# jason-li-831202/Vehicle-CV-ADAS

Hardware: AMD Instinct MI355X
Metric: frames/sec end-to-end (detect+lane+NMS+track) per GPU; conv MFMA util % (higher is better)
Workload: dtype fp16x3

## Files before the change

include/adas_hip.h:

```cpp
#ifndef ADAS_HIP_H
#define ADAS_HIP_H
#include <stddef.h>
#include <stdint.h>

#ifdef __cplusplus
extern "C" {
#endif

typedef enum {
    ADAS_OK = 0,
    ADAS_ERR_INVALID = -1,
    ADAS_ERR_IO = -2,
    ADAS_ERR_FORMAT = -3,
    ADAS_ERR_HIP = -4,
    ADAS_ERR_CAPACITY = -5,
    ADAS_ERR_NO_DEVICE = -6
} adas_status;

const char* adas_last_error(void);
int adas_version(void);
int adas_device_count(void);
int adas_set_device(int index);
int adas_device_pci_bus_id(int index, char* out, int out_len);
int adas_malloc(void** d_ptr, size_t bytes);
// ... 42 lines not shown
int adas_engine_ml_info(const adas_engine* e, int batch, int32_t* n_launches, int32_t* n_layers, int32_t* n_items);
int adas_engine_ml_status(const adas_engine* e, int batch, uint32_t* error_word);
int adas_engine_launch_count(adas_engine* e, int batch);
int adas_engine_ml_counters(const adas_engine* e, int batch, int launch, uint32_t head16[16]);
typedef struct adas_ml_view {
    uint64_t buf;
    int32_t cs, coff, c, h, w;
} adas_ml_view;
typedef struct adas_ml_layer_desc {
    int32_t kernel, stride, act, res_mode, up_c, halo_bn;
    adas_ml_view x, y, res, up;
} adas_ml_layer_desc;
int adas_debug_ml_plan(const adas_ml_layer_desc* layers, int n_layers, int batch, int precision, int32_t* deps, int32_t* targets,
                       uint64_t* items, int items_cap, int32_t summary[4]);
int adas_debug_conv_route(const adas_ml_layer_desc* layer, int batch, int precision, char* name, int name_cap);
#define ADAS_PLAN_COLS 29
int adas_engine_plan(const adas_engine* e, int64_t* rows, int rows_cap, int32_t* n_ops, uint64_t* weight_bytes);
int adas_debug_engine_plan(const void* tables, size_t bytes, int precision, int max_batch, int64_t* rows, int rows_cap, int32_t* n_ops,
                           uint64_t* weight_bytes);
#define ADAS_LABEL_CAP 96
int adas_engine_schedule(const adas_engine* e, int batch, int32_t* step_of, int32_t* role, int cap, int32_t* n_ops, int32_t* n_steps);
int adas_debug_engine_schedule(const void* tables, size_t bytes, int precision, int max_batch, int batch, int32_t* step_of, int32_t* role,
                               char* labels, int cap, int32_t* n_ops, int32_t* n_steps);
int adas_engine_fetch_activation(adas_engine* e, int layer, int batch, float* h_out_nchw, int64_t dims[4]);

int adas_preprocess_yolo(const uint8_t* d_frames_bgr, int n, int src_h, int src_w, float* d_out_nchw, int dst_h,
                         int dst_w, int keep_ratio, void* stream);
int adas_preprocess_ufld(const uint8_t* d_frames_bgr, int n, int src_h, int src_w, float* d_out_nchw, int in_h,
                         int in_w, double crop_ratio, void* stream);
int adas_preprocess_yolo_packed(const uint8_t* d_frames_bgr, int n, int src_h, int src_w, uint16_t* d_out_nhwc4, int dst_h,
// ... 507 lines not shown
```

vehicle-cv-adas_amd/_lib.py:

```python
import ctypes as C
import os

import numpy as np

HERE = os.path.dirname(os.path.abspath(__file__))
LIB_PATH = os.environ.get("ADAS_LIB") or os.path.join(HERE, "libadas_hip.so")

UFLD_MAX_POINTS = 128
HEAD_V8, HEAD_V5, HEAD_V5_LITE = 0, 1, 2
NMS_REFERENCE, NMS_GREEDY = 0, 1
PREC_BF16, PREC_FP32, PREC_FP16, PREC_FP16X3 = 0, 1, 2, 3
PRECISIONS = {"bf16": PREC_BF16, "fp32": PREC_FP32, "fp16": PREC_FP16, "fp16x3": PREC_FP16X3}


class AdasError(RuntimeError):
    def __init__(self, code, msg):
        super().__init__(f"libadas_hip error {code}: {msg}")
        self.code = code


class YoloPostParams(C.Structure):
    _fields_ = [("layout", C.c_int32), ("num_anchors", C.c_int32), ("num_classes", C.c_int32), ("nms_mode", C.c_int32),
                ("box_score", C.c_double), ("iou_thr", C.c_double), ("pad_h", C.c_int32), ("pad_w", C.c_int32),
                ("ratio_h", C.c_double), ("ratio_w", C.c_double), ("max_candidates", C.c_int32), ("reserved", C.c_int32)]
# ... 197 lines not shown
    "adas_engine_num_outputs": (C.c_int, [_P]),
    "adas_engine_output_shape": (C.c_int, [_P, C.c_int, C.POINTER(C.c_int64), C.POINTER(C.c_int)]),
    "adas_engine_output_name": (C.c_char_p, [_P, C.c_int]),
    "adas_engine_infer_host": (C.c_int, [_P, _P, C.c_int, C.POINTER(_P)]),
    "adas_engine_infer_device": (C.c_int, [_P, _P, C.c_int, _P]),
    "adas_engine_accepts_packed_input": (C.c_int, [_P]),
    "adas_engine_precision": (C.c_int, [_P]),
    "adas_engine_prepare": (C.c_int, [_P, C.c_int]),
    "adas_engine_ml_info": (C.c_int, [_P, C.c_int, C.POINTER(C.c_int32), C.POINTER(C.c_int32), C.POINTER(C.c_int32)]),
    "adas_engine_ml_status": (C.c_int, [_P, C.c_int, C.POINTER(C.c_uint32)]),
    "adas_engine_launch_count": (C.c_int, [_P, C.c_int]),
    "adas_engine_ml_counters": (C.c_int, [_P, C.c_int, C.c_int, C.POINTER(C.c_uint32)]),
    "adas_debug_ml_plan": (C.c_int, [C.POINTER(MlLayerDesc), C.c_int, C.c_int, C.c_int, C.POINTER(C.c_int32), C.POINTER(C.c_int32), C.POINTER(C.c_uint64),
                                     C.c_int, C.POINTER(C.c_int32)]),
    "adas_debug_conv_route": (C.c_int, [C.POINTER(MlLayerDesc), C.c_int, C.c_int, C.c_char_p, C.c_int]),
    "adas_engine_plan": (C.c_int, [_P, C.POINTER(C.c_int64), C.c_int, C.POINTER(C.c_int32), C.POINTER(C.c_uint64)]),
    "adas_debug_engine_plan": (C.c_int, [C.c_char_p, C.c_size_t, C.c_int, C.c_int, C.POINTER(C.c_int64), C.c_int, C.POINTER(C.c_int32), C.POINTER(C.c_uint64)]),
    "adas_engine_schedule": (C.c_int, [_P, C.c_int, C.POINTER(C.c_int32), C.POINTER(C.c_int32), C.c_int, C.POINTER(C.c_int32), C.POINTER(C.c_int32)]),
    "adas_debug_engine_schedule": (C.c_int, [C.c_char_p, C.c_size_t, C.c_int, C.c_int, C.c_int, C.POINTER(C.c_int32), C.POINTER(C.c_int32), C.c_char_p,
                                             C.c_int, C.POINTER(C.c_int32), C.POINTER(C.c_int32)]),
    "adas_engine_model_io_half": (C.c_int, [_P]),
    "adas_engine_infer_device_packed": (C.c_int, [_P, _P, C.c_int, _P]),
    "adas_engine_output_device": (_P, [_P, C.c_int]),
    "adas_engine_stats": (C.c_int, [_P, C.POINTER(C.c_double), C.POINTER(C.c_double), C.POINTER(C.c_int)]),
    "adas_engine_profile": (C.c_int, [_P, _P, C.c_int, C.c_int, _P, C.c_int, C.POINTER(C.c_int)]),
    "adas_engine_layer_info": (C.c_int, [_P, C.c_int, C.c_char_p, C.c_int, C.POINTER(C.c_double), C.POINTER(C.c_int)]),
    "adas_engine_layer_kernel": (C.c_int, [_P, C.c_int, C.c_int, C.c_char_p, C.c_int]),
    "adas_engine_fetch_activation": (C.c_int, [_P, C.c_int, C.c_int, _P, C.POINTER(C.c_int64)]),
    "adas_preprocess_yolo": (C.c_int, [_P, C.c_int, C.c_int, C.c_int, _P, C.c_int, C.c_int, C.c_int, _P]),
    "adas_preprocess_ufld": (C.c_int, [_P, C.c_int, C.c_int, C.c_int, _P, C.c_int, C.c_int, C.c_double, _P]),
# ... 257 lines not shown
```

vehicle-cv-adas_amd/csrc/conv_halo8_x3.hip:

```cpp
#include "kernels.h"
#include "elem16.h"
#include <stdlib.h>
#include <string.h>
#include <type_traits>

namespace adas {

typedef __attribute__((ext_vector_type(4))) float yf32x4;
typedef __attribute__((ext_vector_type(4))) uint32_t yu32x4;
typedef __attribute__((ext_vector_type(2))) uint32_t yu32x2;
typedef __attribute__((address_space(3))) void* ylds_vp;

struct H8XDev {
    const void* in;
    const void* wgt;
    const float* bias;
    void* out;
    const void* res;
    uint32_t in_bytes, wgt_bytes, out_bytes, res_bytes;
    int in_cs, in_coff, cin, H, W;
    int out_cs, out_coff, cout;
    int res_cs, res_coff, res_mode;
    int nck;
    int SW, NS, TPS, WW;
// ... 67 lines not shown
constexpr int X8_NBIAS = 2, X8_NRES = 8;
#endif

#ifdef ADAS_H8X_PROF
__device__ unsigned long long g_h8x_prof[256][32];
#define H8XP(i)                                     \
    if (lane == 0 && grp == 0) {                    \
        const unsigned long long t__ = clock64();   \
        pacc__[i] += t__ - tprev__;                 \
        tprev__ = t__;                              \
    }
#else
#define H8XP(i)
#endif

__host__ __device__ constexpr int x8s_issued(bool lo, int k, int nwp) { return ((lo ? k >= 3 : (k >= 0 && k < 3)) ? 1 : 0) + ((k >= 1 && k <= nwp) ? 1 : 0); }
__host__ __device__ constexpr int x8s_allow(bool lo, int k, int nwp) { return x8s_issued(lo, k, nwp) + x8s_issued(lo, k - 1, nwp) + x8s_issued(lo, k - 2, nwp); }

template <int ACT, int MODE, bool LH, bool SH, int NWP>
__global__ __launch_bounds__(X8_THR, 1) void conv_h8x3_kernel(H8XDev a) {
    static_assert(!SH || (MODE == 2 && !LH), "shared weight tiles: one barrier per tap row, whole tiles");
    static_assert(NWP >= 1 && NWP <= X8_NWP && (SH || NWP == X8_NWP), "window pieces per wave");
    Fp16::enter();
    typedef Fp16::vec8 hvec8;
    constexpr int LOOK = x8_look(MODE);
    extern __shared__ __attribute__((aligned(16))) uint8_t lds8[];

    const int tid = threadIdx.x, lane = tid & 63;
    const int wave = __builtin_amdgcn_readfirstlane(tid >> 6);
    const int lrow = lane & 15, kg = lane >> 4;
// ... 244 lines not shown
            tap(std::integral_constant<int, 3>{}); tap(std::integral_constant<int, 4>{}); tap(std::integral_constant<int, 5>{});
            tap(std::integral_constant<int, 6>{}); tap(std::integral_constant<int, 7>{}); tap(std::integral_constant<int, 8>{});
#ifdef ADAS_H8X_PROF
            if (lastc) { H8XP(3) } else if (islo) { H8XP(2) } else { H8XP(1) }
#endif
        };
        for (int c = 0; c + 1 < a.nck; ++c) {
            if (c & 1) chunk(std::false_type{}, std::true_type{}, c);
            else chunk(std::false_type{}, std::false_type{}, c);
        }
        chunk(std::true_type{}, std::true_type{}, a.nck - 1);

        __builtin_amdgcn_s_waitcnt(0x0F70);
        H8XP(4)
#if !defined(ADAS_H8X_SCALAR_EPI) && !defined(ADAS_H8X_NARROW_ST)
        auto write_out = [&](auto rm_c) {
            constexpr int RM = decltype(rm_c)::value;
            yf32x2 val[4][2][2];
#pragma unroll
            for (int j = 0; j < 4; ++j)
#pragma unroll
                for (int i = 0; i < 2; ++i) {
                    yf32x2 v0 = yf32x2{acc[i + 2][j][0], acc[i + 2][j][1]} * kX3Down + yf32x2{acc[i][j][0], acc[i][j][1]};
                    yf32x2 v1 = yf32x2{acc[i + 2][j][2], acc[i + 2][j][3]} * kX3Down + yf32x2{acc[i][j][2], acc[i][j][3]};
                    if (RM != RES_NONE) {
                        const auto q0 = __builtin_amdgcn_permlane16_swap(rraw[j][i].x, rraw[j][i].z, false, false);
                        const auto q1 = __builtin_amdgcn_permlane16_swap(rraw[j][i].y, rraw[j][i].w, false, false);
                        const yf32x2 r0 = x8_join2(q0[0], q0[1]), r1 = x8_join2(q1[0], q1[1]);
                        if (RM == RES_BEFORE_ACT) { v0 = x8_act2<ACT>(v0 + r0); v1 = x8_act2<ACT>(v1 + r1); }
                        else { v0 = x8_act2<ACT>(v0) + r0; v1 = x8_act2<ACT>(v1) + r1; }
                    } else {
                        v0 = x8_act2<ACT>(v0); v1 = x8_act2<ACT>(v1);
                    }
                    val[j][i][0] = v0; val[j][i][1] = v1;
                    acc[i][j] = yf32x4{biasn[i].x, biasn[i].y, biasn[i].z, biasn[i].w};
                    acc[i + 2][j] = yf32x4{0.f, 0.f, 0.f, 0.f};
                }
            uint32_t hw[4][2][2];
            x8_hi_mode(true);
#pragma unroll
            for (int j = 0; j < 4; ++j)
#pragma unroll
                for (int i = 0; i < 2; ++i) {
                    hw[j][i][0] = x8_cvt_hi2(val[j][i][0]);
                    hw[j][i][1] = x8_cvt_hi2(val[j][i][1]);
                }
            x8_hi_mode(false);
#pragma unroll
            for (int j = 0; j < 4; ++j) {
                const uint32_t oo = po[j] == X8_OOB ? X8_OOB : (po[j] * (uint32_t)a.out_cs + (uint32_t)a.out_coff) * 4u + ch0;
#pragma unroll
                for (int i = 0; i < 2; ++i) {
                    const uint32_t oi = (cb * 64 + hb * 32 + i * 16 + (kg >> 1) * 8 < a.cout) ? oo + i * 64 : X8_OOB;
                    const uint32_t l0 = x8_lo2(val[j][i][0], hw[j][i][0]), l1 = x8_lo2(val[j][i][1], hw[j][i][1]);
                    const auto s0 = __builtin_amdgcn_permlane16_swap(hw[j][i][0], l0, false, false);
                    const auto s1 = __builtin_amdgcn_permlane16_swap(hw[j][i][1], l1, false, false);
                    __builtin_amdgcn_raw_buffer_store_b128(yu32x4{s0[0], s1[0], s0[1], s1[1]}, rout, oi, 0, 0);
                }
            }
        };
#else
        auto write_out = [&](auto rm_c) {
            constexpr int RM = decltype(rm_c)::value;
#pragma unroll
            for (int j = 0; j < 4; ++j) {
                const uint32_t oo = po[j] == X8_OOB ? X8_OOB : (po[j] * (uint32_t)a.out_cs + (uint32_t)a.out_coff) * 4u + ch0;
#pragma unroll
                for (int i = 0; i < 2; ++i) {
#ifdef ADAS_H8X_NARROW_ST
                    const uint32_t oi = (cb * 64 + hb * 32 + i * 16 + kg * 4 < a.cout) ? oo + i * 64 : X8_OOB;
#else
                    const uint32_t oi = (cb * 64 + hb * 32 + i * 16 + (kg >> 1) * 8 < a.cout) ? oo + i * 64 : X8_OOB;
#endif
                    float v[4];
#pragma unroll
// ... 59 lines not shown
#pragma unroll
        for (int i = 0; i < NWP; ++i) gcur[i] = gnxt[i];
        wcur = wnxt_item;
        par = (par + a.nck) & 1;
    }
    if (MODE == 1 && !hb) __builtin_amdgcn_s_barrier();
#ifdef ADAS_H8X_PROF
    if (lane == 0 && grp == 0) {
        unsigned long long* b__ = g_h8x_prof[blockIdx.x & 255];
        for (int i__ = 0; i__ < 16; ++i__)
            if (i__ != 7) atomicAdd(&b__[i__ + 16 * hb], pacc__[i__]);
        atomicAdd(&b__[7 + 16 * hb], (unsigned long long)nit__);
    }
#endif
}

#ifdef ADAS_H8X_PROF
extern "C" int adas_debug_h8x_prof(unsigned long long* out32, int reset) {
    static unsigned long long h[256][32];
    if (out32) {
        if (hipMemcpyFromSymbol(h, HIP_SYMBOL(g_h8x_prof), sizeof(h)) != hipSuccess) return -1;
        for (int i = 0; i < 32; ++i) {
            out32[i] = 0;
            for (int b = 0; b < 256; ++b) out32[i] += h[b][i];
        }
    }
    if (reset) {
        memset(h, 0, sizeof(h));
        if (hipMemcpyToSymbol(HIP_SYMBOL(g_h8x_prof), h, sizeof(h)) != hipSuccess) return -1;
    }
// ... 130 lines not shown
    static bool attr_done = false;
    if (!attr_done) {
        (void)hipFuncSetAttribute((const void*)conv_h8x3_kernel<ACT_NONE, MODE, LH, false, X8_NWP>, hipFuncAttributeMaxDynamicSharedMemorySize, 160 * 1024);
        (void)hipFuncSetAttribute((const void*)conv_h8x3_kernel<ACT_SILU, MODE, LH, false, X8_NWP>, hipFuncAttributeMaxDynamicSharedMemorySize, 160 * 1024);
        (void)hipFuncSetAttribute((const void*)conv_h8x3_kernel<ACT_RELU, MODE, LH, false, X8_NWP>, hipFuncAttributeMaxDynamicSharedMemorySize, 160 * 1024);
        (void)hipFuncSetAttribute((const void*)conv_h8x3_kernel<ACT_LEAKY, MODE, LH, false, X8_NWP>, hipFuncAttributeMaxDynamicSharedMemorySize, 160 * 1024);
        attr_done = true;
    }
    if (act == ACT_SILU) hipLaunchKernelGGL((conv_h8x3_kernel<ACT_SILU, MODE, LH, false, X8_NWP>), grid, dim3(X8_THR), X8_LDS, st, d);
    else if (act == ACT_RELU) hipLaunchKernelGGL((conv_h8x3_kernel<ACT_RELU, MODE, LH, false, X8_NWP>), grid, dim3(X8_THR), X8_LDS, st, d);
    else if (act == ACT_LEAKY) hipLaunchKernelGGL((conv_h8x3_kernel<ACT_LEAKY, MODE, LH, false, X8_NWP>), grid, dim3(X8_THR), X8_LDS, st, d);
    else hipLaunchKernelGGL((conv_h8x3_kernel<ACT_NONE, MODE, LH, false, X8_NWP>), grid, dim3(X8_THR), X8_LDS, st, d);
    return hipGetLastError();
}

hipError_t launch_conv_halo8_x3(const ConvArgs& a, hipStream_t st) {
    HaloPlan pl;
    if (!a.wgt_h8x3 || !halo8_x3_applicable(a) || !x8_plan(a.out.h, a.out.w, &pl)) return hipErrorInvalidValue;
    {
        static int sw = -1;
        if (sw < 0) { const char* e = getenv("ADAS_H8X_SW"); sw = e ? atoi(e) : 0; }
        HaloPlan alt;
        if (sw > 0 && plan_halo_sw(a.out.h, a.out.w, 1, sw, X8_MAXPIX, &alt) && alt.eff >= 0.6) {
            const long nt = (long)a.n * alt.NS * alt.TPS;
            if (x8_blocks_per_unit((nt + 7) / 8, x8_cout_pad(a.out.c) / 64) > 0) pl = alt;
        }
    }
    H8XDev d;
    d.in = a.in.p; d.wgt = a.wgt_h8x3; d.bias = a.bias; d.out = a.out.p; d.res = a.res.p;
    d.in_cs = a.in.cs; d.in_coff = a.in.coff; d.cin = a.in.c; d.H = a.in.h; d.W = a.in.w;
    d.out_cs = a.out.cs; d.out_coff = a.out.coff; d.cout = a.out.c;
    d.res_cs = a.res.cs; d.res_coff = a.res.coff; d.res_mode = a.res_mode;
    d.nck = 2 * (x8_cin_pad(a.in.c) / 32);
    d.in_bytes = (uint32_t)((size_t)a.n * a.in.h * a.in.w * a.in.cs * 4);
    d.wgt_bytes = (uint32_t)halo8_x3_weight_bytes(a.out.c, a.in.c);
    d.out_bytes = (uint32_t)((size_t)a.n * a.out.h * a.out.w * a.out.cs * 4);
    d.res_bytes = a.res_mode != RES_NONE ? (uint32_t)((size_t)a.n * a.out.h * a.out.w * a.res.cs * 4) : 0u;
    d.SW = pl.SW; d.NS = pl.NS; d.TPS = pl.TPS; d.WW = pl.WW;
    d.mg_ww = pl.mg_ww; d.mg_sw = pl.mg_sw;
    d.mg_img = (uint32_t)(((1ull << 32) + (uint64_t)(pl.NS * pl.TPS) - 1) / (uint64_t)(pl.NS * pl.TPS));
    d.mg_tps = (uint32_t)(((1ull << 32) + (uint64_t)pl.TPS - 1) / (uint64_t)pl.TPS);
    d.ntiles = a.n * pl.NS * pl.TPS;
    d.tiles8 = (d.ntiles + 7) / 8;
    d.ncb = x8_cout_pad(a.out.c) / 64;
    d.cpw = x8_blocks_per_unit(d.tiles8, d.ncb);
    if (d.cpw <= 0) return hipErrorInvalidValue;
    const int upt = d.ncb / d.cpw;
    d.mg_upt = (uint32_t)(((1ull << 32) + (uint64_t)upt - 1) / (uint64_t)upt);
    const int units8 = d.tiles8 * upt;
    static int max_slots = -1;
    if (max_slots < 0) { const char* e = getenv("ADAS_H8X_SLOTS"); max_slots = e ? atoi(e) : X8_SLOTS; if (max_slots < 8 || max_slots > 4096) max_slots = X8_SLOTS; }
    const int slots = units8 < max_slots ? units8 : max_slots;
    dim3 grid(8 * slots);
    const int forced = x8_mode();
    const bool pingpong = forced == 3;
    if (x8_share() && forced != 3) {
        const int nwp = (pl.maxpix + 127) / 128;
        if (nwp <= 3) return x8_launch_sh<3>(d, a.act, grid, st);
        if (nwp == 4) return x8_launch_sh<4>(d, a.act, grid, st);
        return x8_launch_sh<5>(d, a.act, grid, st);
    }
    if (x8_lhalf()) return pingpong ? x8_launch<1, true>(d, a.act, grid, st) : x8_launch<2, true>(d, a.act, grid, st);
    return pingpong ? x8_launch<1, false>(d, a.act, grid, st) : x8_launch<2, false>(d, a.act, grid, st);
}

}
```

vehicle-cv-adas_amd/csrc/engine.cpp:

```cpp
#include "engine.h"
#include <string.h>
#include <string>
#include <vector>

using namespace adas;

int adas::free_engine(adas_engine* e) {
    if (!e) return ADAS_OK;
    for (auto& kv : e->schedules) free_schedule(&kv.second);
    e->schedules.clear();
    for (auto& b : e->bufs)
        if (b.d && b.alias_of < 0) (void)hipFree(b.d);
    if (e->d_weights) (void)hipFree(e->d_weights);
    if (e->d_input) (void)hipFree(e->d_input);
    for (auto& ev : e->events)
        if (ev) (void)hipEventDestroy(ev);
    delete e;
    return ADAS_OK;
}

extern "C" {

int adas_engine_destroy(adas_engine* e) { return free_engine(e); }

// ... 370 lines not shown
    }
    return ADAS_OK;
}

int adas_debug_conv_route(const adas_ml_layer_desc* layer, int batch, int precision, char* name, int name_cap) {
    ADAS_REQUIRE(layer && batch > 0 && precision >= PREC_BF16 && precision <= PREC_X3 && name && name_cap > 0, ADAS_ERR_INVALID,
                 "adas_debug_conv_route: bad argument");
    ConvArgs a = conv_args_of_desc(*layer, batch, precision);
    const ConvPlan pl = plan_conv(precision, a.kh, a.kw, a.stride, a.pad, a.max_n, a.res_mode, a.in, a.out);
    a.kpad = pl.kpad;
    if (wants_x3h8_packing(precision, pl.kernel, a.kh, a.kw, a.stride, a.pad, a.res_mode, a.in, a.out)) a.wgt_h8x3 = (const void*)(uintptr_t)0x1000;
    snprintf(name, name_cap, "%s", conv_kernel_name(a));
    return ADAS_OK;
}

int adas_engine_precision(const adas_engine* e) { return e ? e->prec : -1; }
int adas_engine_model_io_half(const adas_engine* e) { return e ? (int)((e->hdr.in_cpad >> 16) & 1u) : 0; }

int adas_engine_accepts_packed_input(const adas_engine* e) {
    return (e && e->prec != PREC_X3 && e->ops.size() >= 2 && e->ops[0].skip && e->ops[1].kernel == CONV_STEM) ? 1 : 0;
}

int adas_engine_infer_device_packed(adas_engine* e, const uint16_t* d_input_nhwc4, int batch, void* stream) {
    ADAS_REQUIRE(e && d_input_nhwc4 && batch > 0 && batch <= e->max_batch, ADAS_ERR_INVALID, "adas_engine_infer_device_packed: bad argument");
    ADAS_REQUIRE(adas_engine_accepts_packed_input(e), ADAS_ERR_INVALID,
                 "this engine's first layer is not the fused stem (fp32 mode or ADAS_NO_STEM): feed the fp32 NCHW tensor instead");
    e->last = (hipStream_t)stream;
    return engine_forward(e, reinterpret_cast<const float*>(d_input_nhwc4), batch, (hipStream_t)stream, true);
}

// ... 109 lines not shown
```

vehicle-cv-adas_amd/csrc/kernels.h:

```cpp
#pragma once
#include <hip/hip_runtime.h>
#include <stdint.h>

namespace adas {

enum { PREC_BF16 = 0, PREC_FP32 = 1, PREC_FP16 = 2, PREC_X3 = 3 };
inline bool prec_is16(int prec) { return prec == PREC_BF16 || prec == PREC_FP16; }
inline int prec_esize(int prec) { return prec_is16(prec) ? 2 : 4; }
enum { ACT_NONE = 0, ACT_SILU = 1, ACT_RELU = 2, ACT_LEAKY = 3 ,
       ACT_HSWISH = 4 , ACT_HSIGMOID = 5 , ACT_RELU6 = 6  };
enum { RES_NONE = 0, RES_AFTER_ACT = 1, RES_BEFORE_ACT = 2 };

int persist_slots(int which);

struct TView {
    void* p;
    int cs, coff, c;
    int h, w;
    int f32;
};

struct ConvArgs {
    TView in, out, res;
    const void* wgt;
// ... 65 lines not shown
hipError_t launch_conv_c2f16_x3(const TView& x, const TView& out, const void* const w[4], const float* const b[4], int n, hipStream_t st);
hipError_t launch_conv_c2f16(const TView& x, const TView& out, const void* w_cv1, const float* b_cv1, const void* w_a, const float* b_a, const void* w_b,
                             const float* b_b, const void* w_cv2, const float* b_cv2, int n, int prec, hipStream_t st);
bool pw_applicable(int prec, int kh, int kw, int stride, int pad, int res_mode, const TView& in, const TView& out);
bool pwg_applicable(const ConvArgs& a);
hipError_t launch_conv_pwg(const ConvArgs& a, hipStream_t st);
const char* pwg_kernel_name(int m, int cout);
hipError_t launch_conv_x3(const ConvArgs& a, hipStream_t st);
const char* conv_x3_kernel_name(const ConvArgs& a);
hipError_t launch_pack_weights_x3(const float* src, void* dst, int cout, int cout_pad, int taps, int cin, int cin_pad, int kpad, hipStream_t st);
bool halo8_x3_shape_ok(int kh, int kw, int stride, int pad, const TView& in, const TView& out);
bool halo8_x3_applicable(const ConvArgs& a);
size_t halo8_x3_weight_bytes(int cout, int cin);
hipError_t launch_pack_weights_h8x3(const float* src, void* dst, int cout, int cin, hipStream_t st);
hipError_t launch_conv_halo8_x3(const ConvArgs& a, hipStream_t st);
hipError_t launch_conv(const ConvArgs& a, hipStream_t st);
const char* conv_kernel_name(const ConvArgs& a, bool stem = false);

hipError_t launch_input_nchw(const float* nchw, TView out, int n, int c_true, int prec, hipStream_t st);
hipError_t launch_maxpool(TView in, TView out, int n, int k, int s, int p, int prec, hipStream_t st);
hipError_t launch_avgpool(TView in, TView out, int n, int k, int s, int p, int prec, hipStream_t st);
hipError_t launch_upsample2(TView in, TView out, int n, int prec, hipStream_t st);
bool depth2space_supported(const TView& in, const TView& out);
hipError_t launch_depth2space(TView in, TView out, int n, int prec, hipStream_t st);
hipError_t launch_detect_v6(const TView* ins, float* out, int n, int nc, int A, const int strides[3], hipStream_t st);
hipError_t launch_detect_v6_dfl(const TView* ins, float* out, int n, int nc, int A, const int strides[3], hipStream_t st);
bool sppf_pool3_applicable(int prec, const TView& in, const TView out[3]);
hipError_t launch_sppf_pool3(const TView& in, const TView out[3], int n, int prec, hipStream_t st);
hipError_t launch_detect_v8(const TView* ins, float* out, int n, int nc, int A, const int strides[3], hipStream_t st);
hipError_t launch_detect_v8_fused(const TView* hidden, const void* const* wfrag, const float* const* bias, float* out, int n, int nc, int A,
// ... 67 lines not shown
```

Measured before the change: 5562.

## Add one-pass halo8 x3 conv kernel with double-buffered input window

Adds a new 3x3 fp16x3 halo conv kernel variant that keeps two full input windows in LDS (up to 160 KB) and a six-slot weight ring. It streams the next tile's window and weights while the current chunk's MFMAs run, replacing the shared-window path for tiles of up to 384 pixels. The epilogue is moved into a shared device function. The aim is to hide input-window reload latency and cut barriers between tiles and channel blocks, at the cost of one block per CU from the large LDS footprint and more complex scheduling. It is on by default and can be disabled with an environment variable.

```diff
diff --git a/include/adas_hip.h b/include/adas_hip.h
--- a/include/adas_hip.h
+++ b/include/adas_hip.h
@@ -80,6 +80,7 @@
 int adas_debug_ml_plan(const adas_ml_layer_desc* layers, int n_layers, int batch, int precision, int32_t* deps, int32_t* targets,
                        uint64_t* items, int items_cap, int32_t summary[4]);
 int adas_debug_conv_route(const adas_ml_layer_desc* layer, int batch, int precision, char* name, int name_cap);
+int adas_debug_h8x3_onepass(const adas_ml_layer_desc* layer, int batch);
 #define ADAS_PLAN_COLS 29
 int adas_engine_plan(const adas_engine* e, int64_t* rows, int rows_cap, int32_t* n_ops, uint64_t* weight_bytes);
 int adas_debug_engine_plan(const void* tables, size_t bytes, int precision, int max_batch, int64_t* rows, int rows_cap, int32_t* n_ops,
diff --git a/vehicle-cv-adas_amd/_lib.py b/vehicle-cv-adas_amd/_lib.py
--- a/vehicle-cv-adas_amd/_lib.py
+++ b/vehicle-cv-adas_amd/_lib.py
@@ -235,6 +235,7 @@
     "adas_debug_ml_plan": (C.c_int, [C.POINTER(MlLayerDesc), C.c_int, C.c_int, C.c_int, C.POINTER(C.c_int32), C.POINTER(C.c_int32), C.POINTER(C.c_uint64),
                                      C.c_int, C.POINTER(C.c_int32)]),
     "adas_debug_conv_route": (C.c_int, [C.POINTER(MlLayerDesc), C.c_int, C.c_int, C.c_char_p, C.c_int]),
+    "adas_debug_h8x3_onepass": (C.c_int, [C.POINTER(MlLayerDesc), C.c_int]),
     "adas_engine_plan": (C.c_int, [_P, C.POINTER(C.c_int64), C.c_int, C.POINTER(C.c_int32), C.POINTER(C.c_uint64)]),
     "adas_debug_engine_plan": (C.c_int, [C.c_char_p, C.c_size_t, C.c_int, C.c_int, C.POINTER(C.c_int64), C.c_int, C.POINTER(C.c_int32), C.POINTER(C.c_uint64)]),
     "adas_engine_schedule": (C.c_int, [_P, C.c_int, C.POINTER(C.c_int32), C.POINTER(C.c_int32), C.c_int, C.POINTER(C.c_int32), C.POINTER(C.c_int32)]),
diff --git a/vehicle-cv-adas_amd/csrc/conv_halo8_x3.hip b/vehicle-cv-adas_amd/csrc/conv_halo8_x3.hip
--- a/vehicle-cv-adas_amd/csrc/conv_halo8_x3.hip
+++ b/vehicle-cv-adas_amd/csrc/conv_halo8_x3.hip
@@ -105,6 +105,55 @@
 #define H8XP(i)
 #endif
 
+#if !defined(ADAS_H8X_SCALAR_EPI) && !defined(ADAS_H8X_NARROW_ST)
+template <int ACT, int RM>
+__device__ __forceinline__ void x8_write_out(const H8XDev& a, __amdgpu_buffer_rsrc_t rout, yf32x4 (&acc)[4][4], const yu32x4 (&rraw)[4][2],
+                                             const float4 (&biasn)[2], const uint32_t (&po)[4], uint32_t ch0, int cb, int hb, int kg) {
+    yf32x2 val[4][2][2];
+#pragma unroll
+    for (int j = 0; j < 4; ++j)
+#pragma unroll
+        for (int i = 0; i < 2; ++i) {
+            yf32x2 v0 = yf32x2{acc[i + 2][j][0], acc[i + 2][j][1]} * kX3Down + yf32x2{acc[i][j][0], acc[i][j][1]};
+            yf32x2 v1 = yf32x2{acc[i + 2][j][2], acc[i + 2][j][3]} * kX3Down + yf32x2{acc[i][j][2], acc[i][j][3]};
+            if (RM != RES_NONE) {
+                const auto q0 = __builtin_amdgcn_permlane16_swap(rraw[j][i].x, rraw[j][i].z, false, false);
+                const auto q1 = __builtin_amdgcn_permlane16_swap(rraw[j][i].y, rraw[j][i].w, false, false);
+                const yf32x2 r0 = x8_join2(q0[0], q0[1]), r1 = x8_join2(q1[0], q1[1]);
+                if (RM == RES_BEFORE_ACT) { v0 = x8_act2<ACT>(v0 + r0); v1 = x8_act2<ACT>(v1 + r1); }
+                else { v0 = x8_act2<ACT>(v0) + r0; v1 = x8_act2<ACT>(v1) + r1; }
+            } else {
+                v0 = x8_act2<ACT>(v0); v1 = x8_act2<ACT>(v1);
+            }
+            val[j][i][0] = v0; val[j][i][1] = v1;
+            acc[i][j] = yf32x4{biasn[i].x, biasn[i].y, biasn[i].z, biasn[i].w};
+            acc[i + 2][j] = yf32x4{0.f, 0.f, 0.f, 0.f};
+        }
+    uint32_t hw[4][2][2];
+    x8_hi_mode(true);
+#pragma unroll
+    for (int j = 0; j < 4; ++j)
+#pragma unroll
+        for (int i = 0; i < 2; ++i) {
+            hw[j][i][0] = x8_cvt_hi2(val[j][i][0]);
+            hw[j][i][1] = x8_cvt_hi2(val[j][i][1]);
+        }
+    x8_hi_mode(false);
+#pragma unroll
+    for (int j = 0; j < 4; ++j) {
+        const uint32_t oo = po[j] == X8_OOB ? X8_OOB : (po[j] * (uint32_t)a.out_cs + (uint32_t)a.out_coff) * 4u + ch0;
+#pragma unroll
+        for (int i = 0; i < 2; ++i) {
+            const uint32_t oi = (cb * 64 + hb * 32 + i * 16 + (kg >> 1) * 8 < a.cout) ? oo + i * 64 : X8_OOB;
+            const uint32_t l0 = x8_lo2(val[j][i][0], hw[j][i][0]), l1 = x8_lo2(val[j][i][1], hw[j][i][1]);
+            const auto s0 = __builtin_amdgcn_permlane16_swap(hw[j][i][0], l0, false, false);
+            const auto s1 = __builtin_amdgcn_permlane16_swap(hw[j][i][1], l1, false, false);
+            __builtin_amdgcn_raw_buffer_store_b128(yu32x4{s0[0], s1[0], s0[1], s1[1]}, rout, oi, 0, 0);
+        }
+    }
+}
+#endif
+
 __host__ __device__ constexpr int x8s_issued(bool lo, int k, int nwp) { return ((lo ? k >= 3 : (k >= 0 && k < 3)) ? 1 : 0) + ((k >= 1 && k <= nwp) ? 1 : 0); }
 __host__ __device__ constexpr int x8s_allow(bool lo, int k, int nwp) { return x8s_issued(lo, k, nwp) + x8s_issued(lo, k - 1, nwp) + x8s_issued(lo, k - 2, nwp); }
 
@@ -379,51 +428,7 @@
         __builtin_amdgcn_s_waitcnt(0x0F70);
         H8XP(4)
 #if !defined(ADAS_H8X_SCALAR_EPI) && !defined(ADAS_H8X_NARROW_ST)
-        auto write_out = [&](auto rm_c) {
-            constexpr int RM = decltype(rm_c)::value;
-            yf32x2 val[4][2][2];
-#pragma unroll
-            for (int j = 0; j < 4; ++j)
-#pragma unroll
-                for (int i = 0; i < 2; ++i) {
-                    yf32x2 v0 = yf32x2{acc[i + 2][j][0], acc[i + 2][j][1]} * kX3Down + yf32x2{acc[i][j][0], acc[i][j][1]};
-                    yf32x2 v1 = yf32x2{acc[i + 2][j][2], acc[i + 2][j][3]} * kX3Down + yf32x2{acc[i][j][2], acc[i][j][3]};
-                    if (RM != RES_NONE) {
-                        const auto q0 = __builtin_amdgcn_permlane16_swap(rraw[j][i].x, rraw[j][i].z, false, false);
-                        const auto q1 = __builtin_amdgcn_permlane16_swap(rraw[j][i].y, rraw[j][i].w, false, false);
-                        const yf32x2 r0 = x8_join2(q0[0], q0[1]), r1 = x8_join2(q1[0], q1[1]);
-                        if (RM == RES_BEFORE_ACT) { v0 = x8_act2<ACT>(v0 + r0); v1 = x8_act2<ACT>(v1 + r1); }
-                        else { v0 = x8_act2<ACT>(v0) + r0; v1 = x8_act2<ACT>(v1) + r1; }
-                    } else {
-                        v0 = x8_act2<ACT>(v0); v1 = x8_act2<ACT>(v1);
-                    }
-                    val[j][i][0] = v0; val[j][i][1] = v1;
-                    acc[i][j] = yf32x4{biasn[i].x, biasn[i].y, biasn[i].z, biasn[i].w};
-                    acc[i + 2][j] = yf32x4{0.f, 0.f, 0.f, 0.f};
-                }
-            uint32_t hw[4][2][2];
-            x8_hi_mode(true);
-#pragma unroll
-            for (int j = 0; j < 4; ++j)
-#pragma unroll
-                for (int i = 0; i < 2; ++i) {
-                    hw[j][i][0] = x8_cvt_hi2(val[j][i][0]);
-                    hw[j][i][1] = x8_cvt_hi2(val[j][i][1]);
-                }
-            x8_hi_mode(false);
-#pragma unroll
-            for (int j = 0; j < 4; ++j) {
-                const uint32_t oo = po[j] == X8_OOB ? X8_OOB : (po[j] * (uint32_t)a.out_cs + (uint32_t)a.out_coff) * 4u + ch0;
-#pragma unroll
-                for (int i = 0; i < 2; ++i) {
-                    const uint32_t oi = (cb * 64 + hb * 32 + i * 16 + (kg >> 1) * 8 < a.cout) ? oo + i * 64 : X8_OOB;
-                    const uint32_t l0 = x8_lo2(val[j][i][0], hw[j][i][0]), l1 = x8_lo2(val[j][i][1], hw[j][i][1]);
-                    const auto s0 = __builtin_amdgcn_permlane16_swap(hw[j][i][0], l0, false, false);
-                    const auto s1 = __builtin_amdgcn_permlane16_swap(hw[j][i][1], l1, false, false);
-                    __builtin_amdgcn_raw_buffer_store_b128(yu32x4{s0[0], s1[0], s0[1], s1[1]}, rout, oi, 0, 0);
-                }
-            }
-        };
+        auto write_out = [&](auto rm_c) { x8_write_out<ACT, decltype(rm_c)::value>(a, rout, acc, rraw, biasn, po, ch0, cb, hb, kg); };
 #else
         auto write_out = [&](auto rm_c) {
             constexpr int RM = decltype(rm_c)::value;
@@ -513,6 +518,311 @@
     }
 #endif
 }
+
+#if !defined(ADAS_H8X_SCALAR_EPI) && !defined(ADAS_H8X_NARROW_ST)
+#define ADAS_H8X_HAS_ONEPASS 1
+constexpr int O8_MAXPIX = 384;
+constexpr int O8_WIN = O8_MAXPIX * 128;
+constexpr int O8_NWP = O8_MAXPIX / 8 / 8;
+constexpr int O8_RING = 6;
+constexpr int O8_WR = 2 * O8_WIN;
+constexpr int O8_LDS = O8_WR + O8_RING * X8_TAP;
+static_assert(O8_LDS <= 160 * 1024, "LDS of one CU");
+
+__host__ __device__ constexpr int o8_tiles(int k) { return (k >= 0 && k < 9 && k % 3 == 0) ? 3 : 0; }
+__host__ __device__ constexpr int o8_pieces(int k) { return (k >= 0 && k < O8_NWP) ? 1 : 0; }
+__host__ __device__ constexpr int o8_allow(int k) { return o8_pieces(k - 2) + o8_pieces(k - 1) + o8_pieces(k); }
+static_assert(o8_tiles(0) + o8_tiles(3) + o8_tiles(6) == 9 && o8_tiles(1) + o8_tiles(2) + o8_tiles(4) + o8_tiles(5) + o8_tiles(7) + o8_tiles(8) == 0,
+              "nine tiles a chunk, at the first tap of each row");
+static_assert(o8_allow(2) + o8_allow(5) + o8_allow(8) == O8_NWP, "every window piece is in flight across exactly one row wait ...");
+static_assert(o8_allow(8) == 0, "... and none across the chunk's last: the next window is whole when it is read");
+
+template <int ACT>
+__device__ __forceinline__ void x8_onepass_body(const H8XDev& a) {
+    Fp16::enter();
+    typedef Fp16::vec8 hvec8;
+    extern __shared__ __attribute__((aligned(16))) uint8_t lds8[];
+
+    const int tid = threadIdx.x, lane = tid & 63;
+    const int wave = __builtin_amdgcn_readfirstlane(tid >> 6);
+    const int lrow = lane & 15, kg = lane >> 4;
+    const int hb = wave >> 2, grp = wave & 3;
+    const int xcd = blockIdx.x & 7, slot = blockIdx.x >> 3, nslot = gridDim.x >> 3;
+    int tiles_here = a.ntiles - xcd * a.tiles8;
+    tiles_here = tiles_here < 0 ? 0 : (tiles_here > a.tiles8 ? a.tiles8 : tiles_here);
+    const int upt = a.ncb / a.cpw;
+    const int units_here = tiles_here * upt;
+    if (slot >= units_here) return;
+    const int nch = a.nck >> 1;
+
+    __amdgpu_buffer_rsrc_t rin = __builtin_amdgcn_make_buffer_rsrc((void*)a.in, 0, a.in_bytes, 0x00020000);
+    __amdgpu_buffer_rsrc_t rwg = __builtin_amdgcn_make_buffer_rsrc((void*)a.wgt, 0, a.wgt_bytes, 0x00020000);
+    __amdgpu_buffer_rsrc_t rout = __builtin_amdgcn_make_buffer_rsrc((void*)a.out, 0, a.out_bytes, 0x00020000);
+    __amdgpu_buffer_rsrc_t rres = __builtin_amdgcn_make_buffer_rsrc((void*)(a.res_mode != RES_NONE ? a.res : a.out), 0,
+                                                                    a.res_mode != RES_NONE ? a.res_bytes : 0u, 0x00020000);
+    const int per_img = a.NS * a.TPS;
+    const int gsw[4] = {0, 2, 3, 1};
+    const uint32_t wlane = (uint32_t)((lane >> 2) * 64 + (((lane & 3) ^ gsw[(lane >> 4) & 3]) << 4));
+    const uint32_t wpiece = (uint32_t)((lane & 7) ^ ((lane >> 4) & 1) ^ (((lane >> 5) & 1) << 2)) << 4;
+    const uint32_t wrd = (uint32_t)(O8_WR + hb * 4096 + lrow * 64 + ((kg ^ gsw[(lrow >> 2) & 3]) << 4));
+    const uint32_t ch_lane = (uint32_t)((hb * 4 + (kg >> 1)) * 32 + (kg & 1) * 16);
+    const bool has_res = a.res_mode != RES_NONE;
+
+    struct Tile {
+        int img, sx0, p0, y_first;
+    };
+    auto decode = [&](int u) {
+        Tile t;
+        int tile = xcd * a.tiles8 + (upt == 1 ? u : (int)__umulhi((uint32_t)u, a.mg_upt));
+        t.img = per_img == 1 ? tile : (int)__umulhi((uint32_t)tile, a.mg_img);
+        tile -= t.img * per_img;
+        const int strip = a.TPS == 1 ? tile : (int)__umulhi((uint32_t)tile, a.mg_tps);
+        t.sx0 = strip * a.SW;
+        t.p0 = (tile - strip * a.TPS) * X8_BM;
+        t.y_first = (int)(((uint32_t)t.p0 * a.mg_sw) >> 20);
+        return t;
+    };
+    auto win_offset = [&](const Tile& t, int i) {
+        const int y_lastp = (int)(((uint32_t)(t.p0 + X8_BM - 1) * a.mg_sw) >> 20);
+        const int npix = (y_lastp - t.y_first + 3) * a.WW;
+        const int pix = (wave + 8 * i) * 8 + (lane >> 3);
+        const int wy = (int)(((uint32_t)pix * a.mg_ww) >> 20), wx = pix - wy * a.WW;
+        const int iy = t.y_first - 1 + wy, ix = t.sx0 - 1 + wx;
+        const bool ok = pix < npix && (unsigned)iy < (unsigned)a.H && (unsigned)ix < (unsigned)a.W;
+        const uint32_t off = ((uint32_t)((t.img * a.H + iy) * a.W + ix) * (uint32_t)a.in_cs + (uint32_t)a.in_coff) * 4u + wpiece;
+        const uint32_t m = 0u - (uint32_t)ok;
+        return (off & m) | (X8_OOB & ~m);
+    };
+    auto tap00 = [&](const Tile& t, int j) {
+        const int p = t.p0 + (grp * 4 + j) * 16 + lrow;
+        const int y = (int)(((uint32_t)p * a.mg_sw) >> 20), xs = p - y * a.SW;
+        return (uint32_t)((((y - t.y_first) * a.WW + xs) << 7) | (kg << 5));
+    };
+    auto tap_offset = [&](uint32_t ap128, int t) {
+        const uint32_t v = ap128 + (uint32_t)(((t / 3) * a.WW + (t % 3)) << 7);
+        return v ^ ((v >> 4) & 0x10u) ^ ((v >> 3) & 0x40u);
+    };
+    auto out_pixel = [&](const Tile& t, int j) {
+        const int p = t.p0 + (grp * 4 + j) * 16 + lrow;
+        const int y = (int)(((uint32_t)p * a.mg_sw) >> 20), x = t.sx0 + (p - y * a.SW);
+        return (y < a.H && x < a.W) ? (uint32_t)((t.img * a.H + y) * a.W + x) : X8_OOB;
+    };
+    auto wgt_base = [&](int cb) { return (uint32_t)(((2 * cb + hb) * a.nck) * X8_SLAB + grp * 1024); };
+    auto load_bias = [&](int cb, float4* b) {
+#pragma unroll
+        for (int i = 0; i < 2; ++i) b[i] = *reinterpret_cast<const float4*>(a.bias + cb * 64 + hb * 32 + i * 16 + kg * 4);
+    };
+
+    auto first_cb = [&](int u) { return upt == 1 ? 0 : (u - (int)__umulhi((uint32_t)u, a.mg_upt) * upt) * a.cpw; };
+    int ti = slot, cb = first_cb(slot), cbi = 0;
+    Tile cur = decode(ti);
+    uint32_t gcur[O8_NWP], gnxt[O8_NWP];
+    uint32_t xoff[4][9];
+    uint32_t po[4];
+#pragma unroll
+    for (int i = 0; i < O8_NWP; ++i) gcur[i] = win_offset(cur, i);
+#pragma unroll
+    for (int j = 0; j < 4; ++j) {
+        const uint32_t ap128 = tap00(cur, j);
+#pragma unroll
+        for (int t = 0; t < 9; ++t) xoff[j][t] = tap_offset(ap128, t);
+        po[j] = out_pixel(cur, j);
+    }
+    uint32_t wcur = wgt_base(cb);
+    int par = 0;
+    float4 biasn[2];
+    load_bias(cb, biasn);
+
+#pragma unroll
+    for (int i = 0; i < O8_NWP; ++i)
+        __builtin_amdgcn_raw_ptr_buffer_load_lds(rin, (ylds_vp)(lds8 + (wave + 8 * i) * 1024), 16, gcur[i], 0, 0, 0);
+#pragma unroll
+    for (int t = 0; t < 3; ++t)
+        __builtin_amdgcn_raw_ptr_buffer_load_lds(rwg, (ylds_vp)(lds8 + O8_WR + t * X8_TAP + wave * 1024), 16, wlane, wcur + t * 4096, 0, 0);
+    yf32x4 acc[4][4];
+#pragma unroll
+    for (int j = 0; j < 4; ++j) {
+#pragma unroll
+        for (int i = 0; i < 2; ++i) {
+            acc[i][j] = yf32x4{biasn[i].x, biasn[i].y, biasn[i].z, biasn[i].w};
+            acc[i + 2][j] = yf32x4{0.f, 0.f, 0.f, 0.f};
+        }
+    }
+    x8_wait_vm<0>();
+    __builtin_amdgcn_s_barrier();
+#ifdef ADAS_H8X_PROF
+    unsigned long long tprev__ = clock64();
+    unsigned long long pacc__[16] = {0, 0, 0, 0, 0, 0, 0, 0, 0, 0, 0, 0, 0, 0, 0, 0};
+    int nit__ = 0;
+#endif
+
+    for (;;) {
+        H8XP(0)
+        const bool newtile = cbi + 1 == a.cpw;
+        const bool has_next = !newtile || ti + nslot < units_here;
+        const int cbn = newtile ? first_cb(has_next ? ti + nslot : ti) : cb + 1;
+        const uint32_t ch0 = (uint32_t)(cb * 256) + ch_lane;
+#ifndef ADAS_H8X_NO_TRIM
+        const bool wave_on = cb * 64 + hb * 32 < a.cout;
+#else
+        constexpr bool wave_on = true;
+#endif
+        Tile nxt = cur;
+        uint32_t wnxt_item = 0, apn[4] = {0, 0, 0, 0};
+        yu32x4 rraw[4][2];
+
+        auto chunk = [&](auto last_c, const int c) {
+            constexpr bool lastc = decltype(last_c)::value;
+            if (lastc) {
+                if (newtile && has_next) nxt = decode(ti + nslot);
+                if (!has_next) nxt.y_first = a.H + 4;
+                wnxt_item = wgt_base(cbn);
+#pragma unroll
+                for (int j = 0; j < 4; ++j) apn[j] = tap00(nxt, j);
+                gnxt[0] = win_offset(nxt, 0);
+            } else {
+#pragma unroll
+                for (int i = 0; i < O8_NWP; ++i) gcur[i] += 128u;
+            }
+            const uint32_t wthis = wcur + (uint32_t)(2 * c) * X8_SLAB;
+            const uint32_t wnext = lastc ? wnxt_item : wthis + 2u * X8_SLAB;
+            const int pc = (par + c) & 1;
+            const uint32_t winr = (uint32_t)(pc * O8_WIN), winw = O8_WIN - winr;
+            const uint32_t ringa = (uint32_t)(pc * 3 * X8_TAP), ringb = 3 * X8_TAP - ringa;
+            auto tap = [&](auto kk_c) {
+                constexpr int kk = decltype(kk_c)::value;
+                constexpr int row = kk / 3, col = kk % 3;
+                if constexpr (col == 0) {
+                    const uint32_t src = row < 2 ? wthis + (uint32_t)(kk + 3) * 4096u : wnext;
+                    const uint32_t dst = (uint32_t)O8_WR + (row == 1 ? ringa : ringb) + (uint32_t)wave * 1024u;
+#pragma unroll
+                    for (int m = 0; m < 3; ++m)
+                        __builtin_amdgcn_raw_ptr_buffer_load_lds(rwg, (ylds_vp)(lds8 + dst + m * X8_TAP), 16, wlane, src + (uint32_t)m * 4096u, 0, 0);
+                }
+                if constexpr (kk < O8_NWP)
+                    __builtin_amdgcn_raw_ptr_buffer_load_lds(rin, (ylds_vp)(lds8 + winw + (wave + 8 * kk) * 1024), 16, lastc ? gnxt[kk] : gcur[kk], 0, 0, 0);
+                if (lastc && kk == X8_RES_TAP) {
+                    __builtin_amdgcn_sched_barrier(0);
+                    load_bias(cbn, biasn);
+                    if (has_res) {
+#pragma unroll
+                        for (int j = 0; j < 4; ++j) {
+                            const uint32_t ro = po[j] == X8_OOB ? X8_OOB : (po[j] * (uint32_t)a.res_cs + (uint32_t)a.res_coff) * 4u + ch0;
+#pragma unroll
+                            for (int i = 0; i < 2; ++i) {
+                                const uint32_t ri = (cb * 64 + hb * 32 + i * 16 + (kg >> 1) * 8 < a.cout) ? ro + i * 64 : X8_OOB;
+                                rraw[j][i] = __builtin_bit_cast(yu32x4, __builtin_amdgcn_raw_buffer_load_b128(rres, ri, 0, 0));
+                            }
+                        }
+                    }
+                    __builtin_amdgcn_sched_barrier(0);
+                }
+                hvec8 wf[4], xh[4], xl[4];
+                if (wave_on) {
+                    const uint32_t wsl = wrd + (row == 1 ? ringb : ringa) + (uint32_t)(col * X8_TAP);
+#pragma unroll
+                    for (int i = 0; i < 4; ++i) wf[i] = *reinterpret_cast<const hvec8*>(lds8 + wsl + i * 1024);
+#pragma unroll
+                    for (int j = 0; j < 4; ++j) xh[j] = *reinterpret_cast<const hvec8*>(lds8 + xoff[j][kk] + winr);
+#pragma unroll
+                    for (int j = 0; j < 4; ++j) xl[j] = *reinterpret_cast<const hvec8*>(lds8 + (xoff[j][kk] ^ 16u) + winr);
+                }
+                if constexpr (col == 2) {
+#ifdef ADAS_H8X_ONEPASS_DRAIN
+                    x8_wait_vm<0>();
+#else
+                    constexpr bool with_res = lastc && X8_RES_TAP / 3 == row;
+                    if (with_res && has_res) x8_wait_vm<o8_allow(kk) + X8_NBIAS + X8_NRES>();
+                    else if (with_res) x8_wait_vm<o8_allow(kk) + X8_NBIAS>();
+                    else x8_wait_vm<o8_allow(kk)>();
+#endif
+                }
+                __builtin_amdgcn_s_setprio(1);
+                if (lastc) {
+#pragma unroll
+                    for (int j = 0; j < 4; ++j) xoff[j][kk] = tap_offset(apn[j], kk);
+                    if constexpr (kk + 1 < O8_NWP) gnxt[kk + 1] = win_offset(nxt, kk + 1);
+                }
+                if (wave_on) {
+#pragma unroll
+                    for (int i = 0; i < 2; ++i)
+#pragma unroll
+                        for (int j = 0; j < 4; ++j) acc[i][j] = Fp16::mfma(wf[i], xh[j], acc[i][j]);
+#pragma unroll
+                    for (int i = 0; i < 2; ++i)
+#pragma unroll
+                        for (int j = 0; j < 4; ++j) acc[i + 2][j] = Fp16::mfma(wf[i + 2], xh[j], acc[i + 2][j]);
+#pragma unroll
+                    for (int i = 0; i < 2; ++i)
+#pragma unroll
+                        for (int j = 0; j < 4; ++j) acc[i + 2][j] = Fp16::mfma(wf[i], xl[j], acc[i + 2][j]);
+                }
+                if (lastc) {
+#pragma unroll
+                    for (int g = 0; g < 24; ++g) {
+                        __builtin_amdgcn_sched_group_barrier(0x008, 1, 0);
+                        __builtin_amdgcn_sched_group_barrier(0x006, 4, 0);
+                    }
+                }
+                __builtin_amdgcn_s_setprio(0);
+                if constexpr (col == 2) {
+                    __builtin_amdgcn_sched_barrier(0);
+                    __builtin_amdgcn_s_barrier();
+                    __builtin_amdgcn_sched_barrier(0);
+                }
+            };
+            tap(std::integral_constant<int, 0>{}); tap(std::integral_constant<int, 1>{}); tap(std::integral_constant<int, 2>{});
+            tap(std::integral_constant<int, 3>{}); tap(std::integral_constant<int, 4>{}); tap(std::integral_constant<int, 5>{});
+            tap(std::integral_constant<int, 6>{}); tap(std::integral_constant<int, 7>{}); tap(std::integral_constant<int, 8>{});
+#ifdef ADAS_H8X_PROF
+            if (lastc) { H8XP(3) } else { H8XP(1) }
+#endif
+        };
+        for (int c = 0; c + 1 < nch; ++c) chunk(std::false_type{}, c);
+        chunk(std::true_type{}, nch - 1);
+
+        __builtin_amdgcn_s_waitcnt(0x0F70);
+        H8XP(4)
+        if (a.res_mode == RES_NONE) x8_write_out<ACT, RES_NONE>(a, rout, acc, rraw, biasn, po, ch0, cb, hb, kg);
+        else if (a.res_mode == RES_BEFORE_ACT) x8_write_out<ACT, RES_BEFORE_ACT>(a, rout, acc, rraw, biasn, po, ch0, cb, hb, kg);
+        else x8_write_out<ACT, RES_AFTER_ACT>(a, rout, acc, rraw, biasn, po, ch0, cb, hb, kg);
+        H8XP(5)
+#ifdef ADAS_H8X_PROF
+        ++nit__;
+#endif
+
+        if (!has_next) break;
+        if (newtile) {
+            ti += nslot;
+            cur = nxt;
+#pragma unroll
+            for (int j = 0; j < 4; ++j) po[j] = out_pixel(cur, j);
+        }
+        cb = cbn;
+        cbi = newtile ? 0 : cbi + 1;
+#pragma unroll
+        for (int i = 0; i < O8_NWP; ++i) gcur[i] = gnxt[i];
+        wcur = wnxt_item;
+        par = (par + nch) & 1;
+    }
+#ifdef ADAS_H8X_PROF
+    if (lane == 0 && grp == 0) {
+        unsigned long long* b__ = g_h8x_prof[blockIdx.x & 255];
+        for (int i__ = 0; i__ < 16; ++i__)
+            if (i__ != 7) atomicAdd(&b__[i__ + 16 * hb], pacc__[i__]);
+        atomicAdd(&b__[7 + 16 * hb], (unsigned long long)nit__);
+    }
+#endif
+}
+#define X8_ONEPASS_KERNEL(ACT) \
+    template <>                \
+    __global__ __launch_bounds__(X8_THR, 1) void conv_h8x3_kernel<ACT, 3, false, true, 3>(H8XDev a) { x8_onepass_body<ACT>(a); }
+X8_ONEPASS_KERNEL(ACT_NONE)
+X8_ONEPASS_KERNEL(ACT_SILU)
+X8_ONEPASS_KERNEL(ACT_RELU)
+X8_ONEPASS_KERNEL(ACT_LEAKY)
+#undef X8_ONEPASS_KERNEL
+#endif
 
 #ifdef ADAS_H8X_PROF
 extern "C" int adas_debug_h8x_prof(unsigned long long* out32, int reset) {
@@ -673,18 +983,60 @@
     return hipGetLastError();
 }
 
+static bool x8_onepass_on() {
+    static int v = -1;
+    if (v < 0) {
+        const char* e = getenv("ADAS_H8X_ONEPASS");
+        v = e ? atoi(e) : 1;
+    }
+    return v != 0;
+}
+
+static bool x8_launch_plan(const ConvArgs& a, HaloPlan* pl) {
+    if (!a.wgt_h8x3 || !halo8_x3_applicable(a) || !x8_plan(a.out.h, a.out.w, pl)) return false;
+    static int sw = -1;
+    if (sw < 0) { const char* e = getenv("ADAS_H8X_SW"); sw = e ? atoi(e) : 0; }
+    HaloPlan alt;
+    if (sw > 0 && plan_halo_sw(a.out.h, a.out.w, 1, sw, X8_MAXPIX, &alt) && alt.eff >= 0.6) {
+        const long nt = (long)a.n * alt.NS * alt.TPS;
+        if (x8_blocks_per_unit((nt + 7) / 8, x8_cout_pad(a.out.c) / 64) > 0) *pl = alt;
+    }
+    return true;
+}
+
+bool halo8_x3_onepass(const ConvArgs& a) {
+#ifdef ADAS_H8X_HAS_ONEPASS
+    HaloPlan pl;
+    if (!x8_onepass_on() || !x8_share() || x8_mode() == 3) return false;
+    if (!x8_launch_plan(a, &pl)) return false;
+    return (pl.maxpix + 127) / 128 <= 3 && pl.maxpix <= O8_MAXPIX;
+#else
+    (void)a;
+    return false;
+#endif
+}
+
+#ifdef ADAS_H8X_HAS_ONEPASS
+static hipError_t x8_launch_onepass(const H8XDev& d, int act, dim3 grid, hipStream_t st) {
+    static bool attr_done = false;
+    if (!attr_done) {
+        (void)hipFuncSetAttribute((const void*)conv_h8x3_kernel<ACT_NONE, 3, false, true, 3>, hipFuncAttributeMaxDynamicSharedMemorySize, 160 * 1024);
+        (void)hipFuncSetAttribute((const void*)conv_h8x3_kernel<ACT_SILU, 3, false, true, 3>, hipFuncAttributeMaxDynamicSharedMemorySize, 160 * 1024);
+        (void)hipFuncSetAttribute((const void*)conv_h8x3_kernel<ACT_RELU, 3, false, true, 3>, hipFuncAttributeMaxDynamicSharedMemorySize, 160 * 1024);
+        (void)hipFuncSetAttribute((const void*)conv_h8x3_kernel<ACT_LEAKY, 3, false, true, 3>, hipFuncAttributeMaxDynamicSharedMemorySize, 160 * 1024);
+        attr_done = true;
+    }
+    if (act == ACT_SILU) hipLaunchKernelGGL((conv_h8x3_kernel<ACT_SILU, 3, false, true, 3>), grid, dim3(X8_THR), O8_LDS, st, d);
+    else if (act == ACT_RELU) hipLaunchKernelGGL((conv_h8x3_kernel<ACT_RELU, 3, false, true, 3>), grid, dim3(X8_THR), O8_LDS, st, d);
+    else if (act == ACT_LEAKY) hipLaunchKernelGGL((conv_h8x3_kernel<ACT_LEAKY, 3, false, true, 3>), grid, dim3(X8_THR), O8_LDS, st, d);
+    else hipLaunchKernelGGL((conv_h8x3_kernel<ACT_NONE, 3, false, true, 3>), grid, dim3(X8_THR), O8_LDS, st, d);
+    return hipGetLastError();
+}
+#endif
+
 hipError_t launch_conv_halo8_x3(const ConvArgs& a, hipStream_t st) {
     HaloPlan pl;
-    if (!a.wgt_h8x3 || !halo8_x3_applicable(a) || !x8_plan(a.out.h, a.out.w, &pl)) return hipErrorInvalidValue;
-    {
-        static int sw = -1;
-        if (sw < 0) { const char* e = getenv("ADAS_H8X_SW"); sw = e ? atoi(e) : 0; }
-        HaloPlan alt;
-        if (sw > 0 && plan_halo_sw(a.out.h, a.out.w, 1, sw, X8_MAXPIX, &alt) && alt.eff >= 0.6) {
-            const long nt = (long)a.n * alt.NS * alt.TPS;
-            if (x8_blocks_per_unit((nt + 7) / 8, x8_cout_pad(a.out.c) / 64) > 0) pl = alt;
-        }
-    }
+    if (!x8_launch_plan(a, &pl)) return hipErrorInvalidValue;
     H8XDev d;
     d.in = a.in.p; d.wgt = a.wgt_h8x3; d.bias = a.bias; d.out = a.out.p; d.res = a.res.p;
     d.in_cs = a.in.cs; d.in_coff = a.in.coff; d.cin = a.in.c; d.H = a.in.h; d.W = a.in.w;
@@ -713,6 +1065,9 @@
     dim3 grid(8 * slots);
     const int forced = x8_mode();
     const bool pingpong = forced == 3;
+#ifdef ADAS_H8X_HAS_ONEPASS
+    if (halo8_x3_onepass(a)) return x8_launch_onepass(d, a.act, grid, st);
+#endif
     if (x8_share() && forced != 3) {
         const int nwp = (pl.maxpix + 127) / 128;
         if (nwp <= 3) return x8_launch_sh<3>(d, a.act, grid, st);
diff --git a/vehicle-cv-adas_amd/csrc/engine.cpp b/vehicle-cv-adas_amd/csrc/engine.cpp
--- a/vehicle-cv-adas_amd/csrc/engine.cpp
+++ b/vehicle-cv-adas_amd/csrc/engine.cpp
@@ -408,6 +408,15 @@
     return ADAS_OK;
 }
 
+int adas_debug_h8x3_onepass(const adas_ml_layer_desc* layer, int batch) {
+    if (!layer || batch <= 0) return -1;
+    ConvArgs a = conv_args_of_desc(*layer, batch, PREC_X3);
+    const ConvPlan pl = plan_conv(PREC_X3, a.kh, a.kw, a.stride, a.pad, a.max_n, a.res_mode, a.in, a.out);
+    a.kpad = pl.kpad;
+    if (wants_x3h8_packing(PREC_X3, pl.kernel, a.kh, a.kw, a.stride, a.pad, a.res_mode, a.in, a.out)) a.wgt_h8x3 = (const void*)(uintptr_t)0x1000;
+    return (conv_route(a) == ConvRoute::H8X3 && halo8_x3_onepass(a)) ? 1 : 0;
+}
+
 int adas_engine_precision(const adas_engine* e) { return e ? e->prec : -1; }
 int adas_engine_model_io_half(const adas_engine* e) { return e ? (int)((e->hdr.in_cpad >> 16) & 1u) : 0; }
 
diff --git a/vehicle-cv-adas_amd/csrc/kernels.h b/vehicle-cv-adas_amd/csrc/kernels.h
--- a/vehicle-cv-adas_amd/csrc/kernels.h
+++ b/vehicle-cv-adas_amd/csrc/kernels.h
@@ -103,6 +103,7 @@
 size_t halo8_x3_weight_bytes(int cout, int cin);
 hipError_t launch_pack_weights_h8x3(const float* src, void* dst, int cout, int cin, hipStream_t st);
 hipError_t launch_conv_halo8_x3(const ConvArgs& a, hipStream_t st);
+bool halo8_x3_onepass(const ConvArgs& a);
 hipError_t launch_conv(const ConvArgs& a, hipStream_t st);
 const char* conv_kernel_name(const ConvArgs& a, bool stem = false);
 
```

Measured after the change: 5707, median of 6. +2.6%, better.
